# L-Forster/Zero-TIG

Measured on AMD Instinct MI355X. Metric: 1080p self-supervised training frames/sec, higher is better.
Workload: dtype bf16; 1 GPU; 1080x1920 BVI-RLV-style self-supervised training step (enhance+RAFT flow+warp+loss+backward+clip+Adam), batch 1 frame per GPU, of_scale=3, dataset=RLV; parallelism=dp1 (one contiguous clip per rank, one 370 KB flat-bucket all-reduce per step), global_batch=1, launch=hipGraph replay, collective=none (single process, no launcher)

## Files before the change

### zero-tig_amd/csrc/zt_conv.h

```cpp
#pragma once
#include "zt_common.h"

constexpr int TH = 4, TW = 32;

__device__ __forceinline__ float apply_act(float v, int act) {
  switch (act) {
    case 1: return fmaxf(v, 0.f);
    case 2: return v > 0.f ? v : 0.2f * v;
    case 3: return 1.f / (1.f + expf(-v));
    case 4: return tanhf(v);
    case 5: return fminf(fmaxf(1.f / (1.f + expf(-v)), 0.0001f), 1.f);
    default: return v;
  }
}

struct ConvArgsH {
  const zt_bf16* x;
  const zt_bf16* x2;
  const zt_bf16* w;
  const float* bias;
  const zt_bf16* aux;
  void* y;
  int N, H, W, Cin, ldx, ldx2, csplit;
  int Ho, Wo, Cout, CoutP, ldk, ldy, ldaux;
  int padH, padW;
  int act, epi, out_mode;
  float alpha;
  int tilesX, tilesY;
  zt_bf16* y2;
  int ldy2, esplit;
  float* stats;
  const zt_bf16* zprev;
  int ldz;
  const float* bn_scale;
  const float* bn_shift;
  const float* bn_mean;
};

constexpr int HCK = 32;

namespace {
__device__ const uint4 zt_zero_chunk = {0u, 0u, 0u, 0u};
}

__device__ __forceinline__ zt_f32x4 zt_mfma_bf16_k16(zt_s16x4 a, zt_s16x4 b, zt_f32x4 c) {
  return __builtin_amdgcn_mfma_f32_16x16x16bf16_1k(a, b, c, 0, 0, 0);
}

#define ZT_HIDDEN __attribute__((visibility("hidden")))
ZT_HIDDEN int zt_launch_conv_tiled(const ConvArgsH& a, int KH, int KW, int stride, int MT, int NT, hipStream_t stream);
ZT_HIDDEN int zt_launch_conv_ws(ConvArgsH& a, int K, int NT, int CCH, hipStream_t stream);
ZT_HIDDEN int zt_launch_conv_rs(ConvArgsH& a, hipStream_t stream);
ZT_HIDDEN int zt_launch_conv1x1_thinout(const ConvArgsH& a, hipStream_t stream);
ZT_HIDDEN int zt_launch_conv1x1_thin(const ConvArgsH& a, hipStream_t stream);
ZT_HIDDEN int zt_launch_wgrad_reduce(const float* slab, int nslab, int ntap, int CT16, int NT16, float* grad_w, int Cout, int Cin,
                                     int accumulate, float* grad_b, hipStream_t stream);

extern "C" int zt_conv2d_nhwc_bf16(const void* x, const void* x2, int csplit, int ldx, int ldx2, int N, int H, int W, int Cin,
                                   const void* w, int CoutP, int ldk, const float* bias, void* y, int ldy, int out_mode, int Cout,
                                   int KH, int KW, int stride, int padH, int padW, int act, float alpha, const void* aux,
                                   int ldaux, int epi, hipStream_t stream);
```

### zero-tig_amd/csrc/zt_conv.hip

```cpp
#include "zt_conv.h"
#include <stdlib.h>

namespace {

constexpr int ZT_MAXREP = 24;
struct RepackTable {
  const float* src[ZT_MAXREP];
  zt_bf16* dst[ZT_MAXREP];
  int Cout[ZT_MAXREP], Cin[ZT_MAXREP], K[ZT_MAXREP], CoutP[ZT_MAXREP], ldk[ZT_MAXREP], tflip[ZT_MAXREP];
};

__global__ void __launch_bounds__(256) repack_w_bf16_multi_kernel(RepackTable t) {
  const int en = blockIdx.y;
  const int Cout = t.Cout[en], Cin = t.Cin[en], KH = t.K[en], KW = t.K[en], CoutP = t.CoutP[en], ldk = t.ldk[en];
  const int total = Cout * Cin * KH * KW;
  for (int idx = blockIdx.x * 256 + threadIdx.x; idx < total; idx += gridDim.x * 256) {
    const int kx = idx % KW, ky = (idx / KW) % KH, ci = (idx / (KW * KH)) % Cin, co = idx / (KW * KH * Cin);
    const zt_bf16 v = zt_f2bf(t.src[en][idx]);
    if (!t.tflip[en]) t.dst[en][((size_t)(ky * KW + kx) * CoutP + co) * ldk + ci] = v;
    else t.dst[en][((size_t)((KH - 1 - ky) * KW + (KW - 1 - kx)) * CoutP + ci) * ldk + co] = v;
  }
}

__global__ void __launch_bounds__(256) repack_w_bf16_kernel(const float* __restrict__ src, zt_bf16* __restrict__ dst, int Cout,
                                                            int Cin, int KH, int KW, int CoutP, int ldk, int co_off,
                                                            int transpose_flip, int total) {
  int idx = blockIdx.x * 256 + threadIdx.x;
  if (idx >= total) return;
  int kx = idx % KW;
  int ky = (idx / KW) % KH;
  int ci = (idx / (KW * KH)) % Cin;
  int co = idx / (KW * KH * Cin);
  zt_bf16 v = zt_f2bf(src[idx]);
  if (!transpose_flip) dst[((size_t)(ky * KW + kx) * CoutP + co_off + co) * ldk + ci] = v;
  else dst[((size_t)((KH - 1 - ky) * KW + (KW - 1 - kx)) * CoutP + co_off + ci) * ldk + co] = v;
}

}

struct BnBwdFuse {
  const void* zprev;
  int ldz;
  const float *scale, *shift, *mean;
};

static int conv2d_bf16_impl(const void* x, const void* x2, int csplit, int ldx, int ldx2, int N, int H, int W, int Cin,
                            const void* w, int CoutP, int ldk, const float* bias, void* y, int ldy, int out_mode,
                            int Cout, int KH, int KW, int stride, int padH, int padW, int act, float alpha,
                            const void* aux, int ldaux, int epi, int variant, void* y2, int ldy2, int esplit, hipStream_t stream,
                            float* stats = nullptr, const BnBwdFuse* bnb = nullptr) {
  ZT_REQUIRE(x && w && y && N > 0 && H > 0 && W > 0 && Cin > 0 && Cout > 0 && out_mode >= 0 && out_mode <= 2);
  ZT_REQUIRE(epi >= 0 && epi <= 6 && (epi < 4 || (out_mode == 0 && variant == 2)) && (epi != 4 || (y2 && esplit > 0 && esplit < Cout)));
  ZT_REQUIRE(ldx % 8 == 0 && ldk % 8 == 0 && ((uintptr_t)x & 15) == 0 && ((uintptr_t)w & 15) == 0);
  ZT_REQUIRE(!x2 || (csplit % HCK == 0 && ldx2 % 8 == 0 && ((uintptr_t)x2 & 15) == 0));
  ZT_REQUIRE(epi == 0 || aux);
  ConvArgsH a;
  a.x = (const zt_bf16*)x; a.x2 = (const zt_bf16*)x2; a.w = (const zt_bf16*)w; a.bias = bias; a.aux = (const zt_bf16*)aux; a.y = y;
  a.N = N; a.H = H; a.W = W; a.Cin = Cin; a.ldx = ldx; a.ldx2 = ldx2; a.csplit = csplit;
  a.Ho = (H + 2 * padH - KH) / stride + 1;
  a.Wo = (W + 2 * padW - KW) / stride + 1;
  a.Cout = Cout; a.CoutP = CoutP; a.ldk = ldk; a.ldy = ldy; a.ldaux = ldaux;
  a.padH = padH; a.padW = padW; a.act = act; a.epi = epi; a.out_mode = out_mode; a.alpha = alpha;
  a.y2 = (zt_bf16*)y2; a.ldy2 = ldy2; a.esplit = esplit; a.stats = stats;
  a.zprev = nullptr; a.ldz = 0; a.bn_scale = a.bn_shift = a.bn_mean = nullptr;
  if (bnb) { a.zprev = (const zt_bf16*)bnb->zprev; a.ldz = bnb->ldz; a.bn_scale = bnb->scale; a.bn_shift = bnb->shift; a.bn_mean = bnb->mean; }
  ZT_REQUIRE(variant >= 0 && variant <= 3 && a.Ho > 0 && a.Wo > 0);
  ZT_REQUIRE((long long)N * H * W * (ldx > ldx2 ? ldx : ldx2) < 0x7FFFFFFFll && (long long)KH * KW * CoutP * ldk < 0x7FFFFFFFll);
  a.tilesY = zt_cdiv(a.Ho, TH);
  int c16 = (Cout + 15) / 16;
  int NT = c16 >= 4 ? ((c16 % 4 == 0) ? 4 : (c16 % 3 == 0 ? 3 : 4)) : c16;
  int MT = 2;
  long long wgs = (long long)zt_cdiv(a.Wo, 32) * a.tilesY * N * zt_cdiv(c16, NT);
  if (wgs < 512 || stride == 2) MT = 1;
  if (MT == 1 && NT == 4 && (long long)zt_cdiv(a.Wo, 16) * a.tilesY * N * zt_cdiv(c16, NT) < 512 && c16 % 2 == 0) NT = 2;
  if (NT == 4 && c16 % 2 == 0 && stride == 1) NT = 2;
  const bool ws_ok = N == 1 && stride == 1 && KH == KW && (KH == 1 || KH == 3) && padH == KH / 2 && padW == KW / 2 && Cin <= 64 && !x2;
  ZT_REQUIRE(variant != 1 || ws_ok);
  if (variant == 0 && N == 1 && KH == 1 && KW == 1 && stride == 1 && padH == 0 && padW == 0 && !x2 && Cout <= 8 && out_mode == 1 &&
      epi == 0 && Cin % 8 == 0 && Cin <= 64 && ldk >= Cin && CoutP >= Cout) {
    zt_launch_conv1x1_thinout(a, stream);
    ZT_LAUNCH_CHECK();
    return ZT_OK;
  }
  if (variant == 0 && N == 1 && KH == 1 && KW == 1 && stride == 1 && padH == 0 && padW == 0 && !x2 && Cin <= 8 && ldx == 8 && ldk == 8 &&
      out_mode == 0 && act <= 2 && Cout % 8 == 0 && CoutP >= Cout && ldy % 8 == 0 && ((uintptr_t)y & 15) == 0 &&
      (!aux || (ldaux % 8 == 0 && ((uintptr_t)aux & 15) == 0))) {
    zt_launch_conv1x1_thin(a, stream);
    ZT_LAUNCH_CHECK();
    return ZT_OK;
  }
  const bool rs_ok = ws_ok && KH == 3 && out_mode == 0 && act <= 2 && alpha == 1.f && ldy % 8 == 0 && ((uintptr_t)y & 15) == 0 &&
                     (!aux || (ldaux % 8 == 0 && ((uintptr_t)aux & 15) == 0)) && ldx >= 8 &&
                     ((Cout == 64 && (Cin <= 16 || Cin == 56 || Cin == 64)) || (Cout == 48 && (Cin <= 16 || Cin == 40 || Cin == 48)));
  ZT_REQUIRE(variant != 3 || rs_ok);
  if (stats && !(rs_ok && variant == 3)) return ZT_EINVAL;
  if (rs_ok && (variant == 3 || (variant == 0 && (long long)zt_cdiv(a.Wo, TW) * zt_cdiv(a.Ho, 8) >= 1024))) {
    int rcp = zt_launch_conv_rs(a, stream);
    if (rcp) return rcp;
    ZT_LAUNCH_CHECK();
    return ZT_OK;
  }
  if (variant != 2 && ws_ok && (variant == 1 || (long long)zt_cdiv(a.Wo, TW) * zt_cdiv(a.Ho, 8) >= 1024)) {
    a.tilesX = zt_cdiv(a.Wo, TW);
    int CCH = Cin <= 32 ? 1 : 2;
    int rcw = zt_launch_conv_ws(a, KH, NT, CCH, stream);
    if (rcw) return rcw;
    ZT_LAUNCH_CHECK();
    return ZT_OK;
  }
  a.tilesX = zt_cdiv(a.Wo, 16 * MT);
  int rc = zt_launch_conv_tiled(a, KH, KW, stride, MT, NT, stream);
  if (rc) return rc;
  ZT_LAUNCH_CHECK();
  return ZT_OK;
}

extern "C" int zt_conv2d_nhwc_bf16_variant(const void* x, const void* x2, int csplit, int ldx, int ldx2, int N, int H, int W, int Cin,
                                           const void* w, int CoutP, int ldk, const float* bias, void* y, int ldy, int out_mode,
                                           int Cout, int KH, int KW, int stride, int padH, int padW, int act, float alpha,
                                           const void* aux, int ldaux, int epi, int variant, hipStream_t stream) {
  ZT_REQUIRE(epi >= 0 && epi <= 3);
  return conv2d_bf16_impl(x, x2, csplit, ldx, ldx2, N, H, W, Cin, w, CoutP, ldk, bias, y, ldy, out_mode, Cout, KH, KW, stride, padH, padW,
                          act, alpha, aux, ldaux, epi, variant, nullptr, 0, 0, stream);
}

extern "C" int zt_conv2d_nhwc_bf16_ex(const void* x, const void* x2, int csplit, int ldx, int ldx2, int N, int H, int W, int Cin,
                                      const void* w, int CoutP, int ldk, const float* bias, void* y, int ldy, int out_mode,
                                      int Cout, int KH, int KW, int stride, int padH, int padW, int act, float alpha,
                                      const void* aux, int ldaux, int epi, void* y2, int ldy2, int esplit, hipStream_t stream) {
  return conv2d_bf16_impl(x, x2, csplit, ldx, ldx2, N, H, W, Cin, w, CoutP, ldk, bias, y, ldy, out_mode, Cout, KH, KW, stride, padH, padW,
                          act, alpha, aux, ldaux, epi, epi >= 4 ? 2 : 0, y2, ldy2, esplit, stream);
}

extern "C" int zt_chan_stats_nhwc(const void* x, int dt, int ldx, int N, int HW, int C, int nblk, float* partial, hipStream_t stream);

extern "C" int zt_conv3x3_bn_stats_bf16(const void* x, int ldx, int H, int W, int Cin, const void* w, int CoutP, int ldk, const float* bias,
                                        void* y, int ldy, int Cout, float* stats, int stats_blocks, hipStream_t stream) {
  ZT_REQUIRE(x && w && y && stats && stats_blocks == 512 && Cout % 8 == 0);
  hipError_t e = hipMemsetAsync(stats, 0, sizeof(float) * (size_t)stats_blocks * 2 * Cout, stream);
  if (e != hipSuccess) return (int)e;
  const char* mt = getenv("ZT_STATS_FUSE_MIN_TILES");
  const long long min_tiles = mt ? atoll(mt) : 1024;
  const bool fused = Cout == 64 && (Cin == 56 || Cin == 64) && ldx >= 8 && ldy % 8 == 0 && ((uintptr_t)y & 15) == 0 &&
                     (long long)zt_cdiv(W, TW) * zt_cdiv(H, 8) >= min_tiles;
  if (fused)
    return conv2d_bf16_impl(x, nullptr, 0, ldx, 0, 1, H, W, Cin, w, CoutP, ldk, bias, y, ldy, 0, Cout, 3, 3, 1, 1, 1, 0, 1.f, nullptr, 0, 0, 3,
                            nullptr, 0, 0, stream, stats);
  int rc = conv2d_bf16_impl(x, nullptr, 0, ldx, 0, 1, H, W, Cin, w, CoutP, ldk, bias, y, ldy, 0, Cout, 3, 3, 1, 1, 1, 0, 1.f, nullptr, 0, 0, 0,
                            nullptr, 0, 0, stream);
  if (rc) return rc;
  const int HW = H * W;
  int nblk = HW / 64 < 1 ? 1 : (HW / 64 > stats_blocks ? stats_blocks : HW / 64);
  return zt_chan_stats_nhwc(y, 1, ldy, 1, HW, Cout, nblk, stats, stream);
}

extern "C" int zt_conv3x3_dgrad_bn_sums_bf16(const void* dz, int lddz, int H, int W, const void* wT, int CoutP, int ldk, void* df, int lddf,
                                             const void* res, int ldres, const void* zprev, int ldz, const float* bn_scale,
                                             const float* bn_shift, const float* bn_mean, float* stats, int stats_blocks, hipStream_t stream) {
  ZT_REQUIRE(dz && wT && df && res && zprev && bn_scale && bn_shift && bn_mean && stats && stats_blocks == 512);
  ZT_REQUIRE(ldz % 8 == 0 && ((uintptr_t)zprev & 15) == 0 && (long long)zt_cdiv(W, TW) * zt_cdiv(H, 4) >= 1);
  hipError_t e = hipMemsetAsync(stats, 0, sizeof(float) * (size_t)stats_blocks * 2 * 64, stream);
  if (e != hipSuccess) return (int)e;
  BnBwdFuse b = {zprev, ldz, bn_scale, bn_shift, bn_mean};
  return conv2d_bf16_impl(dz, nullptr, 0, lddz, 0, 1, H, W, 64, wT, CoutP, ldk, nullptr, df, lddf, 0, 64, 3, 3, 1, 1, 1, 0, 1.f, res, ldres, 3, 3, nullptr, 0,
                          0, stream, stats, &b);
}

extern "C" int zt_conv2d_nhwc_bf16(const void* x, const void* x2, int csplit, int ldx, int ldx2, int N, int H, int W, int Cin,
                                   const void* w, int CoutP, int ldk, const float* bias, void* y, int ldy, int out_mode, int Cout,
                                   int KH, int KW, int stride, int padH, int padW, int act, float alpha, const void* aux,
                                   int ldaux, int epi, hipStream_t stream) {
  return zt_conv2d_nhwc_bf16_variant(x, x2, csplit, ldx, ldx2, N, H, W, Cin, w, CoutP, ldk, bias, y, ldy, out_mode, Cout, KH, KW,
                                     stride, padH, padW, act, alpha, aux, ldaux, epi, 0, stream);
}

extern "C" int zt_repack_conv_weights_bf16_multi(int n, const void* const* src, void* const* dst, const int* Cout, const int* Cin,
                                                 const int* K, const int* CoutP, const int* ldk, const int* transpose_flip,
                                                 hipStream_t stream) {
  ZT_REQUIRE(n >= 1 && n <= ZT_MAXREP && src && dst && Cout && Cin && K && CoutP && ldk && transpose_flip);
  RepackTable t;
  int maxtotal = 0;
  for (int i = 0; i < ZT_MAXREP; ++i) {
    const int j = i < n ? i : 0;
    ZT_REQUIRE(src[j] && dst[j] && CoutP[j] % 16 == 0 && ldk[j] % 8 == 0);
    t.src[i] = (const float*)src[j]; t.dst[i] = (zt_bf16*)dst[j]; t.Cout[i] = Cout[j]; t.Cin[i] = Cin[j]; t.K[i] = K[j];
    t.CoutP[i] = CoutP[j]; t.ldk[i] = ldk[j]; t.tflip[i] = transpose_flip[j];
    const int total = Cout[j] * Cin[j] * K[j] * K[j];
    if (i < n && total > maxtotal) maxtotal = total;
  }
  int gx = zt_cdiv(maxtotal, 256);
  hipLaunchKernelGGL(repack_w_bf16_multi_kernel, dim3(gx > 64 ? 64 : gx, n), dim3(256), 0, stream, t);
  ZT_LAUNCH_CHECK();
  return ZT_OK;
}

extern "C" int zt_repack_conv_weight_bf16(const float* src, void* dst, int Cout, int Cin, int KH, int KW, int CoutP, int ldk,
                                          int co_off, int transpose_flip, hipStream_t stream) {
  ZT_REQUIRE(src && dst && CoutP % 16 == 0 && ldk % 8 == 0);
  int total = Cout * Cin * KH * KW;
  hipLaunchKernelGGL(repack_w_bf16_kernel, dim3(zt_cdiv(total, 256)), dim3(256), 0, stream, src, (zt_bf16*)dst, Cout, Cin, KH, KW,
                     CoutP, ldk, co_off, transpose_flip, total);
  ZT_LAUNCH_CHECK();
  return ZT_OK;
}
```

Baseline: 116.0 frames/s.

## Add register-streaming thin-input 3x3 conv kernel for Cin<=16 layers

Adds a specialized 3x3 conv kernel for very thin inputs (Cin<=16, Cout 48/64) that keeps all nine weight taps in registers, streams input rows through a register ring with a rolling three-row accumulator, and builds the horizontal taps with lane shuffles instead of shared memory. It is dispatched by default ahead of the existing rs kernel for large images, and an environment variable can turn it off. The aim is to cut the redundant loads and padded-K waste of the generic kernel on first-layer style convs. The cost is higher register pressure and a persistent grid capped at 512 blocks, which could limit occupancy.

```diff
diff --git a/zero-tig_amd/csrc/zt_conv.h b/zero-tig_amd/csrc/zt_conv.h
--- a/zero-tig_amd/csrc/zt_conv.h
+++ b/zero-tig_amd/csrc/zt_conv.h
@@ -51,6 +51,7 @@
 ZT_HIDDEN int zt_launch_conv_tiled(const ConvArgsH& a, int KH, int KW, int stride, int MT, int NT, hipStream_t stream);
 ZT_HIDDEN int zt_launch_conv_ws(ConvArgsH& a, int K, int NT, int CCH, hipStream_t stream);
 ZT_HIDDEN int zt_launch_conv_rs(ConvArgsH& a, hipStream_t stream);
+ZT_HIDDEN int zt_launch_conv_thinin(ConvArgsH& a, hipStream_t stream);
 ZT_HIDDEN int zt_launch_conv1x1_thinout(const ConvArgsH& a, hipStream_t stream);
 ZT_HIDDEN int zt_launch_conv1x1_thin(const ConvArgsH& a, hipStream_t stream);
 ZT_HIDDEN int zt_launch_wgrad_reduce(const float* slab, int nslab, int ntap, int CT16, int NT16, float* grad_w, int Cout, int Cin,
diff --git a/zero-tig_amd/csrc/zt_conv.hip b/zero-tig_amd/csrc/zt_conv.hip
--- a/zero-tig_amd/csrc/zt_conv.hip
+++ b/zero-tig_amd/csrc/zt_conv.hip
@@ -36,6 +36,11 @@
   else dst[((size_t)((KH - 1 - ky) * KW + (KW - 1 - kx)) * CoutP + co_off + ci) * ldk + co] = v;
 }
 
+}
+
+static bool thinin_enabled() {
+  const char* e = getenv("ZT_THININ");
+  return !(e && e[0] == '0');
 }
 
 struct BnBwdFuse {
@@ -64,7 +69,7 @@
   a.y2 = (zt_bf16*)y2; a.ldy2 = ldy2; a.esplit = esplit; a.stats = stats;
   a.zprev = nullptr; a.ldz = 0; a.bn_scale = a.bn_shift = a.bn_mean = nullptr;
   if (bnb) { a.zprev = (const zt_bf16*)bnb->zprev; a.ldz = bnb->ldz; a.bn_scale = bnb->scale; a.bn_shift = bnb->shift; a.bn_mean = bnb->mean; }
-  ZT_REQUIRE(variant >= 0 && variant <= 3 && a.Ho > 0 && a.Wo > 0);
+  ZT_REQUIRE(variant >= 0 && variant <= 4 && a.Ho > 0 && a.Wo > 0);
   ZT_REQUIRE((long long)N * H * W * (ldx > ldx2 ? ldx : ldx2) < 0x7FFFFFFFll && (long long)KH * KW * CoutP * ldk < 0x7FFFFFFFll);
   a.tilesY = zt_cdiv(a.Ho, TH);
   int c16 = (Cout + 15) / 16;
@@ -94,6 +99,14 @@
                      ((Cout == 64 && (Cin <= 16 || Cin == 56 || Cin == 64)) || (Cout == 48 && (Cin <= 16 || Cin == 40 || Cin == 48)));
   ZT_REQUIRE(variant != 3 || rs_ok);
   if (stats && !(rs_ok && variant == 3)) return ZT_EINVAL;
+  const bool ti_ok = rs_ok && Cin <= 16 && Cin <= ldx && (ldx == 8 || ldx == 16) && epi == 0 && !stats && CoutP >= Cout;
+  ZT_REQUIRE(variant != 4 || ti_ok);
+  if (ti_ok && (variant == 4 || (variant == 0 && thinin_enabled() && (long long)zt_cdiv(a.Wo, TW) * zt_cdiv(a.Ho, 8) >= 1024))) {
+    int rct = zt_launch_conv_thinin(a, stream);
+    if (rct) return rct;
+    ZT_LAUNCH_CHECK();
+    return ZT_OK;
+  }
   if (rs_ok && (variant == 3 || (variant == 0 && (long long)zt_cdiv(a.Wo, TW) * zt_cdiv(a.Ho, 8) >= 1024))) {
     int rcp = zt_launch_conv_rs(a, stream);
     if (rcp) return rcp;
diff --git a/zero-tig_amd/csrc/zt_conv_thinin.hip b/zero-tig_amd/csrc/zt_conv_thinin.hip
--- /dev/null
+++ b/zero-tig_amd/csrc/zt_conv_thinin.hip
@@ -0,0 +1,168 @@
+#include "zt_conv.h"
+#include <stdlib.h>
+
+namespace {
+
+constexpr int TI_D = 6;
+constexpr int TI_MAXGRID = 512;
+
+template <int NQ>
+__device__ __forceinline__ int ti_cout(int q, int r) {
+  if (NQ == 3 && q == 2) return 32 + r;
+  return (q >> 1) * 32 + (r >> 2) * 8 + (q & 1) * 4 + (r & 3);
+}
+
+template <int NQ>
+__global__ void __launch_bounds__(256, 2) conv_thinin_bf16_kernel(ConvArgsH a, int nsx, int nseg, int RS) {
+  static_assert(TI_D % 3 == 0, "the accumulator ring has period 3");
+  const int lane = threadIdx.x & 63;
+  const int wave = __builtin_amdgcn_readfirstlane((int)threadIdx.x >> 6);
+  const int l15 = lane & 15, l4 = lane >> 4;
+  const int gw = (int)blockIdx.x * 4 + wave, GW = (int)gridDim.x * 4;
+  const int nitems = nsx * nseg;
+
+  zt_s16x4 wf[9][NQ];
+  zt_f32x4 bq[NQ];
+#pragma unroll
+  for (int q = 0; q < NQ; ++q) {
+    const int kk = l4 * 4 < a.ldk ? l4 * 4 : 0;
+#pragma unroll
+    for (int tap = 0; tap < 9; ++tap) {
+      const zt_bf16* wr = a.w + ((size_t)tap * a.CoutP + ti_cout<NQ>(q, l15)) * a.ldk;
+      const zt_s16x4 v = *reinterpret_cast<const zt_s16x4*>(wr + kk);
+      wf[tap][q] = l4 * 4 < a.ldk ? v : (zt_s16x4){0, 0, 0, 0};
+    }
+#pragma unroll
+    for (int j = 0; j < 4; ++j) bq[q][j] = a.bias ? a.bias[ti_cout<NQ>(q, l4 * 4 + j)] : 0.f;
+  }
+  const float slope = a.act == 0 ? 1.f : (a.act == 1 ? 0.f : 0.2f);
+  const bool has_act = a.act != 0;
+
+  const int cps = a.ldx == 16 ? 1 : 0;
+  const int spix = (lane >> cps) < 17 ? (lane >> cps) : 17;
+  const int schk = lane & ((1 << cps) - 1);
+  unsigned cm[4];
+#pragma unroll
+  for (int d = 0; d < 4; ++d) {
+    const int nv = a.Cin - schk * 8 - 2 * d;
+    cm[d] = nv >= 2 ? ~0u : (nv == 1 ? 0xFFFFu : 0u);
+  }
+  int srcl[3];
+#pragma unroll
+  for (int kx = 0; kx < 3; ++kx) srcl[kx] = ((l15 + kx) << cps) + (cps ? (l4 >> 1) : 0);
+  const bool hi = l4 & 1;
+  const unsigned dmask = (cps || l4 < 2) ? ~0u : 0u;
+
+  for (int item = gw; item < nitems; item += GW) {
+    const int sy = item / nsx, sx = item - sy * nsx;
+    const int x0 = sx * 16, y0 = sy * RS;
+    const int y1 = y0 + RS < a.H ? y0 + RS : a.H;
+    const int nt = y1 - y0 + 2;
+    const int imax = y1 < a.H ? y1 : a.H - 1;
+    const int xx = x0 - 1 + spix;
+    const bool xin = xx >= 0 && xx < a.W;
+    const int soff = (xx < 0 ? 0 : (xx >= a.W ? a.W - 1 : xx)) * a.ldx + schk * 8;
+    unsigned sm[4];
+#pragma unroll
+    for (int d = 0; d < 4; ++d) sm[d] = xin ? cm[d] : 0u;
+    const int ox = x0 + l15;
+    auto load_row = [&](int t, zt_u32x4& dst) {
+      int i = y0 - 1 + t;
+      i = i < 0 ? 0 : (i > imax ? imax : i);
+      const zt_bf16* rp = a.x + (size_t)i * a.W * a.ldx + soff;
+      ZT_HIDDEN_LD16(dst, rp);
+    };
+
+    zt_u32x4 xr[TI_D];
+#pragma unroll
+    for (int s = 0; s < TI_D; ++s) load_row(s, xr[s]);
+    zt_f32x4 acc[3][NQ];
+#pragma unroll
+    for (int s = 0; s < 3; ++s)
+#pragma unroll
+      for (int q = 0; q < NQ; ++q) acc[s][q] = bq[q];
+
+    auto body = [&](int t0, auto big_c) {
+      constexpr bool BIG = decltype(big_c)::value != 0;
+      zt_static_for<0, TI_D>([&](auto u_c) {
+        constexpr int u = decltype(u_c)::value;
+        const int t = t0 + u, i = y0 - 1 + t;
+        ZT_HIDDEN_WAIT4(BIG ? 3 * TI_D - 3 : TI_D - 1, xr[u], sm[0], sm[1], sm[2]);
+        const bool rin = i >= 0 && i < a.H;
+        unsigned r[4];
+#pragma unroll
+        for (int d = 0; d < 4; ++d) r[d] = rin ? (xr[u][d] & sm[d]) : 0u;
+        load_row(t + TI_D, xr[u]);
+        zt_s16x4 f[3];
+#pragma unroll
+        for (int kx = 0; kx < 3; ++kx) {
+          const unsigned g0 = __shfl(r[0], srcl[kx]), g1 = __shfl(r[1], srcl[kx]), g2 = __shfl(r[2], srcl[kx]), g3 = __shfl(r[3], srcl[kx]);
+          uint2 v;
+          v.x = (hi ? g2 : g0) & dmask;
+          v.y = (hi ? g3 : g1) & dmask;
+          f[kx] = __builtin_bit_cast(zt_s16x4, v);
+        }
+        constexpr int s0 = (u + 1) % 3, s1 = u % 3, s2 = (u + 2) % 3;
+#pragma unroll
+        for (int kx = 0; kx < 3; ++kx)
+#pragma unroll
+          for (int q = 0; q < NQ; ++q) {
+            acc[s0][q] = zt_mfma_bf16_k16(wf[kx][q], f[kx], kx == 0 ? bq[q] : acc[s0][q]);
+            acc[s1][q] = zt_mfma_bf16_k16(wf[3 + kx][q], f[kx], acc[s1][q]);
+            acc[s2][q] = zt_mfma_bf16_k16(wf[6 + kx][q], f[kx], acc[s2][q]);
+          }
+        float v[NQ][4];
+#pragma unroll
+        for (int q = 0; q < NQ; ++q)
+#pragma unroll
+          for (int j = 0; j < 4; ++j) v[q][j] = acc[s2][q][j];
+        if (has_act) {
+#pragma unroll
+          for (int q = 0; q < NQ; ++q)
+#pragma unroll
+            for (int j = 0; j < 4; ++j) v[q][j] = ZT_VMAX(v[q][j], slope * v[q][j]);
+        }
+        unsigned pk[NQ][2];
+#pragma unroll
+        for (int q = 0; q < NQ; ++q) {
+          pk[q][0] = zt_f2bf2(v[q][0], v[q][1]);
+          pk[q][1] = zt_f2bf2(v[q][2], v[q][3]);
+        }
+        if (t >= 2 && t < nt && ox < a.W) {
+          zt_bf16* yp = (zt_bf16*)a.y + ((size_t)(i - 1) * a.W + ox) * a.ldy;
+          typedef unsigned u32x2 __attribute__((ext_vector_type(2)));
+          __builtin_nontemporal_store((zt_u32x4){pk[0][0], pk[0][1], pk[1][0], pk[1][1]}, reinterpret_cast<zt_u32x4*>(yp + l4 * 8));
+          if constexpr (NQ == 4) __builtin_nontemporal_store((zt_u32x4){pk[2][0], pk[2][1], pk[3][0], pk[3][1]}, reinterpret_cast<zt_u32x4*>(yp + 32 + l4 * 8));
+          else __builtin_nontemporal_store((u32x2){pk[2][0], pk[2][1]}, reinterpret_cast<u32x2*>(yp + 32 + l4 * 4));
+        }
+      });
+    };
+    int t0 = 0;
+    for (; t0 < nt && t0 < TI_D + 2; t0 += TI_D) body(t0, ZtIdx<0>{});
+    for (; t0 < nt; t0 += TI_D) body(t0, ZtIdx<1>{});
+    ZT_WAIT_HIDDEN_DMA();
+  }
+}
+
+}
+
+int zt_launch_conv_thinin(ConvArgsH& a, hipStream_t stream) {
+  ZT_REQUIRE(a.N == 1 && !a.x2 && a.Cin >= 1 && a.Cin <= 16 && (a.ldx == 8 || a.ldx == 16) && a.Cin <= a.ldx && a.ldk % 8 == 0);
+  ZT_REQUIRE((a.Cout == 48 || a.Cout == 64) && a.CoutP >= a.Cout && a.out_mode == 0 && a.ldy % 8 == 0 && a.ldy >= a.Cout && ((uintptr_t)a.y & 15) == 0);
+  ZT_REQUIRE(a.act >= 0 && a.act <= 2 && a.alpha == 1.f && a.epi == 0 && !a.stats && a.Ho == a.H && a.Wo == a.W);
+  const int nsx = zt_cdiv(a.W, 16);
+  int nseg = TI_MAXGRID * 4 / nsx;
+  if (nseg < 1) nseg = 1;
+  int RS = zt_cdiv(zt_cdiv(a.H, nseg) + 2, TI_D) * TI_D - 2;
+  if (RS < 2 * TI_D - 2) RS = 2 * TI_D - 2;
+  nseg = zt_cdiv(a.H, RS);
+  const long long nitems = (long long)nsx * nseg;
+  ZT_REQUIRE(nitems < 0x7FFFFFFFll);
+  int maxgrid = TI_MAXGRID;
+  if (const char* e = getenv("ZT_THININ_BLOCKS")) maxgrid = atoi(e) > 0 && atoi(e) < TI_MAXGRID ? atoi(e) : maxgrid;
+  const long long wgs = (nitems + 3) / 4;
+  dim3 grid((unsigned)(wgs < maxgrid ? wgs : maxgrid)), block(256);
+  if (a.Cout == 64) hipLaunchKernelGGL((conv_thinin_bf16_kernel<4>), grid, block, 0, stream, a, nsx, nseg, RS);
+  else hipLaunchKernelGGL((conv_thinin_bf16_kernel<3>), grid, block, 0, stream, a, nsx, nseg, RS);
+  return 0;
+}
```

After: 116.8 frames/s, median of 6. About the same (+0.7%).
